# marbl/meryl

Hardware: AMD Instinct MI355X
Metric: distinct k-mers counted/sec (whole node) (higher is better)
Workload: dtype u64; 1 GPU; meryl count k=21 on synthetic short reads: 66666667 x 150 bp reads per GPU (10.00 Gbp per GPU, 30x of a 333333334 bp genome, 0.5% substitutions, 0.01% N), inputs resident in HBM; k=21, reads_per_gpu=66666667, bases_per_gpu=10066666717, n_distinct=1181289506, parallelism=1 GPU, transport=none (one GPU), n_instances=8648488363, w_prefix=18

## Files before the change

meryl_amd/csrc/mgc_api.cpp:

```cpp
#include "../../include/meryl_gpu_count.h"
#include "mgc_device.h"
#include "mgc_session.hpp"
#include "mgc_gzip_par.hpp"
#include "mgc_runs.hpp"
#include "mgc_selector.hpp"
#include "mgc_value.hpp"

#include <algorithm>
#include <cstdio>
#include <cstdlib>
#include <cstring>
#include <string>
#include <thread>
#include <vector>

namespace mgc {
std::string &thread_last_error() {
  thread_local std::string e;
  return e;
}

Switches read_switches() {
  Switches sw;
  auto off = [](const char *n) { const char *e = getenv(n); return e && e[0] == '0'; };
  auto on1 = [](const char *n) { const char *e = getenv(n); return e && e[0] == '1'; };
  auto num = [](const char *n, uint64_t d) { const char *e = getenv(n); return (e && *e) ? strtoull(e, nullptr, 10) : d; };
  sw.fine_hist = !off("MGC_FINE_HIST"); sw.hpc_msd = !off("MGC_HPC_MSD"); sw.hpc_digits = !off("MGC_HPC_DIGITS");
  sw.const_k = !off("MGC_KMER_CONST_K"); sw.packed_bases = !off("MGC_PACKED_BASES"); sw.narrow = !off("MGC_NARROW"); sw.wide_msd = !off("MGC_WIDE_MSD");
  sw.group_pipe = !off("MGC_GROUP_PIPE"); sw.soa5 = !off("MGC_SOA5"); sw.k96 = !off("MGC_K96"); sw.finish = !off("MGC_FINISH");
  sw.nolist = on1("MGC_FINISH_NOLIST");
  sw.finish_trace = getenv("MGC_FINISH_TRACE") != nullptr; sw.group_dbg = getenv("MGC_GROUP_DBG") != nullptr; sw.hash_dbg = getenv("MGC_HASH_DBG") != nullptr;
  { const char *e = getenv("MGC_HASH_MULTI"); sw.hash_multi = (e && *e) ? atoi(e) : -1; }
  { const char *e = getenv("MGC_HASH_STREAM"); sw.hash_stream = (e && *e) ? atoi(e) : -1; }
  sw.min_top = (uint32_t)num("MGC_FINISH_MIN_TOP", 0);
  sw.finish_target = num("MGC_FINISH_TARGET", 0);
  sw.stream_max = num("MGC_STREAM_MAX", (uint64_t)1 << 22);
  sw.bucket_bases = num("MGC_BUCKET_BASES", 0);
  sw.huge_streams = (uint32_t)num("MGC_HUGE_STREAMS", 4);
  sw.huge_slices = !off("MGC_HUGE_SLICES");
  sw.pass_stagger = (uint32_t)num("MGC_PASS_STAGGER", 0);
  sw.group_batch_bytes = num("MGC_GROUP_BATCH_BYTES", sw.group_batch_bytes);
  sw.group_batch_files = (uint32_t)num("MGC_GROUP_BATCH_FILES", 0);
  return sw;
}
}
using mgc::set_err;

namespace {


uint64_t number_of_bits64(uint64_t v) {
  uint64_t b = 0;
  while (v) { b++; v >>= 1; }
  return b;
}

uint64_t expected_simple_size(uint32_t k, uint64_t n_est, uint32_t suffix_len) {
  if (2 * k - 2 * suffix_len > 42) return UINT64_MAX;
  const uint64_t low_bits  = 16;
  const uint64_t n_entries = (uint64_t)1 << (2 * k - 2 * suffix_len);
  const uint64_t exp_max   = (uint64_t)(0.004 * (double)n_est);
  const uint64_t exp_bits  = number_of_bits64(exp_max) + 1;
  const uint64_t extra     = (exp_bits < low_bits) ? 0 : (exp_bits - low_bits);
  return (n_entries * low_bits + n_entries * extra) / 8;
}

void best_prefix_size(const mgc_count_config &c, uint64_t n_est, uint64_t mem_allowed, uint32_t *best,
                      uint64_t *mem_used) {
  const uint32_t k = c.k;
  const uint32_t seg_bits = c.page_size * 8, seg_bytes = c.page_size;
  *best = 0;
  *mem_used = UINT64_MAX;
  for (uint32_t wp = 1; wp < 2 * k - 1; wp++) {
    const uint64_t n_prefix = (uint64_t)1 << wp;
    const uint64_t kpp = n_est / n_prefix + 1;
    const uint64_t kps = seg_bits / (2 * k - wp);
    const uint64_t spp = kpp / kps + 1;
    if (wp + number_of_bits64(spp) + number_of_bits64(seg_bytes) >= 64) break;
    const uint64_t struct_mem = (uint64_t)c.sizeof_count_array * n_prefix + 8 * n_prefix * spp;
    const uint64_t data_min   = n_prefix * seg_bytes;
    const uint64_t total      = struct_mem + n_prefix * spp * seg_bytes;
    if (struct_mem + data_min > mem_allowed) break;
    if ((wp > 9) && (total + (uint64_t)16 * wp * 1024 * 1024 < *mem_used)) {
      *mem_used = total;
      *best = wp;
    }
    if (total > (uint64_t)16 * *mem_used) break;
  }
}

}

extern "C" uint32_t mgc_version(void) { return (0u << 16) | 3u; }

extern "C" int mgc_configure_counting(mgc_count_config *c) {
  if (!c) return MGC_EINVAL;
  if (c->k == 0 || c->k > 64) {
    set_err(nullptr, "ERROR: Kmer size not supplied with modifier k=<kmer-size>.");
    return MGC_EINVAL;
  }
  if (c->mode < 0 || c->mode > 2) return MGC_EINVAL;
  if (c->page_size == 0) c->page_size = 4096;
  if (c->sizeof_count_array == 0) c->sizeof_count_array = 3232;

  c->use_simple = 0; c->w_prefix = 0; c->n_prefix = 0; c->w_data = 0; c->n_batches = 1; c->memory_used = 0;

  const uint64_t mem_simple = expected_simple_size(c->k, c->n_kmers_estimate, c->count_suffix_length);
  uint64_t mem_complex = UINT64_MAX;
  uint32_t best = 0, n_batches = 1;

  if (c->k > 5) {
    for (n_batches = 1; mem_complex > c->memory_allowed; n_batches++) {
      best_prefix_size(*c, c->n_kmers_estimate / n_batches, c->memory_allowed, &best, &mem_complex);
      if (n_batches > (1u << 20)) {
        set_err(nullptr, "configureCounting: no prefix size fits in %lu bytes", (unsigned long)c->memory_allowed);
        return MGC_EINVAL;
      }
    }
    c->w_prefix = best;
    c->n_prefix = (uint64_t)1 << best;
    c->w_data   = 2 * c->k - best;
  }
  if ((mem_simple < mem_complex) && (mem_simple < c->memory_allowed)) {
    c->use_simple = 1; c->memory_used = mem_simple;
  } else {
// ... 1402 lines not shown
```

meryl_amd/csrc/mgc_count.cpp:

```cpp
#include "mgc_session.hpp"
#include "mgc_group_batch.hpp"
#include "mgc_group_route.hpp"

#include <algorithm>
#include <vector>

#define TRY(expr) do { const int rc__ = (expr); if (rc__ != MGC_OK) return rc__; } while (0)

namespace {
using S = mgc_session;

struct StageTimer {
  bool on;
  hipStream_t st;
  hipEvent_t ev[MGC_NUM_STAGES][2];
  bool used[MGC_NUM_STAGES];
  StageTimer(bool enable, hipStream_t s) : on(enable), st(s) {
    for (int i = 0; i < MGC_NUM_STAGES; i++) {
      used[i] = false;
      if (on) { (void)hipEventCreate(&ev[i][0]); (void)hipEventCreate(&ev[i][1]); }
    }
  }
  ~StageTimer() {
    if (on) for (int i = 0; i < MGC_NUM_STAGES; i++) { (void)hipEventDestroy(ev[i][0]); (void)hipEventDestroy(ev[i][1]); }
// ... 316 lines not shown
  std::vector<uint64_t> h_counts(nb);
  const bool wide_msd_on = sw.wide_msd && !c.homopoly_compress;
  if (!in.keys) {
    if (sw.packed_bases && n_bases) {
      const size_t pb = mgc::kp_packed_bytes(n_bases);
      bool room = s->buf[S::B_PACKED].cap >= pb;
      if (!room) {
        size_t free_b = 0, total_b = 0;
        room = hipMemGetInfo(&free_b, &total_b) == hipSuccess &&
               (double)free_b + (double)s->arena_bytes() >= (double)n_bases * (double)(2 + 14ull * kw) + (double)pb;
      }
      if (room) {
        if (s->ensure(S::B_PACKED, pb) == hipSuccess) d_packed = s->buf[S::B_PACKED].p;
        else (void)hipGetLastError();
      }
    }
    tm.begin(MGC_STAGE_HISTOGRAM);
    if (n_bases >= (1u << 22) && ((kw == 1 && 2 * k - bucket_bits <= 41) || wide_msd_on) && mgc::kmer_histogram_fine_ok(k, bucket_bits, s->sfx_mask, sw)) {
      HIP_TRY(s, s->ensure(S::B_FINE, sizeof(uint64_t) << 15));
      uint64_t *fine = reinterpret_cast<uint64_t *>(s->buf[S::B_FINE].p);
      HIP_TRY(s, mgc::launch_kmer_histogram_fine(d_bases, n_bases, k, c.mode, d_counts64, fine, part_ws, st, sw.const_k, 6, d_packed));
      d_fine = fine;
    } else if (c.homopoly_compress && n_bases >= (1u << 22) && (2 * k - bucket_bits) % 2 == 0 && 2 * k - bucket_bits >= 20 &&
               sw.hpc_digits && mgc::kmer_histogram_hpc_ok(k, bucket_bits, s->sfx_mask, sw)) {
      HIP_TRY(s, s->ensure(S::B_FINE, sizeof(uint64_t) * std::max<size_t>((size_t)1 << 15, mgc::kmer_histogram_hpc_entries(bucket_bits))));
      uint64_t *fine = reinterpret_cast<uint64_t *>(s->buf[S::B_FINE].p);
      HIP_TRY(s, mgc::launch_kmer_histogram_hpc(d_bases, n_bases, k, c.mode, bucket_bits, d_counts64, fine, part_ws, st, sw.const_k, d_packed));
      d_fine_hpc = fine;
    } else
    HIP_TRY(s, mgc::launch_kmer_histogram(d_bases, n_bases, k, c.mode, bucket_bits, d_counts64, part_ws, st, s->sfx_mask, s->sfx_test, d_packed));
    tm.end(MGC_STAGE_HISTOGRAM);
    prof.stage_launches[MGC_STAGE_HISTOGRAM] = 1;
    HIP_TRY(s, hipMemcpyAsync(h_counts.data(), d_counts64, sizeof(uint64_t) * nb, hipMemcpyDeviceToHost, st));
    HIP_TRY(s, hipStreamSynchronize(st));
  } else {
    memcpy(h_counts.data(), in.counts, sizeof(uint64_t) * nb);
    uint64_t n_ext = 0;
    for (uint32_t b = 0; b < nb; b++) n_ext += h_counts[b];
    if (in.fine && sw.fine_hist && bucket_bits <= 8 && n_ext >= (1u << 22) && s->sfx_mask == 0 && !c.homopoly_compress &&
        2 * k >= 15 + 2 && ((kw == 1 && 2 * k - bucket_bits <= 41) || wide_msd_on))
      d_fine = in.fine;
  }
  memset(s->file_instances, 0, sizeof(s->file_instances));
  for (uint32_t b = 0; b < nb; b++) {
    plan.files[b].size = h_counts[b];
    plan.files[b].start = h_meta[b] = N;
    N += h_counts[b];
    plan.max_bucket = std::max(plan.max_bucket, h_counts[b]);
    s->file_instances[b >> (bucket_bits - MGC_NUM_FILES_BITS)] += h_counts[b];
  }
  s->n_instances = N;
  plan.fine = d_fine != nullptr;
  plan.fine_hpc = d_fine_hpc != nullptr;
  return MGC_OK;
}

int Count::buffers() {
  mgc::make_sort_plan(0, rem_bits, &full);
  const bool odd = !use_finish && (full.num_passes & 1u) != 0;
  if (!in.keys) HIP_TRY(s, s->ensure(S::B_X, kbytes * N));
  y_base_bytes = kbytes * (odd ? N : plan.max_bucket);
  HIP_TRY(s, s->ensure(S::B_Y, y_base_bytes));
  X = in.keys ? reinterpret_cast<unsigned char *>(in.keys) : reinterpret_cast<unsigned char *>(s->buf[S::B_X].p);
  Y = reinterpret_cast<unsigned char *>(s->buf[S::B_Y].p);
  sort_ws_bytes = mgc::sort_workspace_bytes(plan.max_bucket) + 256;
  HIP_TRY(s, s->ensure(S::B_SORT_WS, sort_ws_bytes));
  sort_ws = s->buf[S::B_SORT_WS].p;
  d_err = reinterpret_cast<uint32_t *>(reinterpret_cast<unsigned char *>(sort_ws) + sort_ws_bytes - 256);
  HIP_TRY(s, hipMemsetAsync(d_err, 0, 32, st));
  if (s->profiling) {
    pass_ev.resize((size_t)nb * ev_per_file);
    for (auto &e : pass_ev) (void)hipEventCreate(&e);
  }
  return MGC_OK;
}

int Count::partition(bool soa, bool k96) {
  if (in.keys) return MGC_OK;
  HIP_TRY(s, hipMemcpyAsync(d_starts, h_meta.data(), sizeof(uint64_t) * nb, hipMemcpyHostToDevice, st));
  uint64_t *d_k96flags = d_starts + nb;
  if (k96) HIP_TRY(s, hipMemcpyAsync(d_k96flags, h_meta.data() + nb, sizeof(uint64_t) * nb, hipMemcpyHostToDevice, st));
  tm.begin(MGC_STAGE_PARTITION);
  HIP_TRY(s, mgc::launch_kmer_partition(d_bases, n_bases, k, c.mode, bucket_bits, d_starts, (void *)X, part_ws, st,
                                        s->sfx_mask, s->sfx_test, k96 ? d_k96flags : (soa ? d_counts64 : nullptr), sw.const_k, d_packed));
  tm.end(MGC_STAGE_PARTITION);
  const uint64_t packed_b = d_packed ? mgc::kp_packed_bytes(n_bases) : 0;
  prof.hist_bytes = n_bases + packed_b;
  prof.partition_bytes = d_packed ? packed_b : n_bases;
  for (uint32_t b = 0; b < nb; b++) prof.partition_bytes += plan.files[b].size * (soa ? 5u : ((k96 && plan.files[b].k96) ? 12u : (uint64_t)kbytes));
  prof.stage_launches[MGC_STAGE_PARTITION] = 2;
  return MGC_OK;
}

int Count::count_full() {
  TRY(partition(false, false));
  const bool odd = (full.num_passes & 1u) != 0;
  tm.begin(MGC_STAGE_SORT);
  for (uint32_t b = 0; b < nb; b++) {
    FilePlan &x = plan.files[b];
    if (x.size == 0) continue;
    void *alt = odd ? (void *)(Y + kbytes * x.start) : (void *)Y;
    int in_alt = 0;
    hipEvent_t *pe = s->profiling ? &pass_ev[(size_t)b * ev_per_file] : nullptr;
    HIP_TRY(s, mgc::launch_radix_sort(seg(b), alt, x.size, kw, full, sort_ws, sort_ws_bytes - 256, d_err, &in_alt, st, pe));
    x.passes = full.num_passes;
    sort_launch_groups++;
  }
  tm.end(MGC_STAGE_SORT);
  void *d_sorted = odd ? (void *)Y : (void *)X;

  HIP_TRY(s, s->ensure(S::B_RLE_WS, mgc::rle_workspace_bytes(N)));
  rle_ws = s->buf[S::B_RLE_WS].p;
  tm.begin(MGC_STAGE_RLE);
  HIP_TRY(s, mgc::launch_rle_count(d_sorted, N, kw, rle_ws, st));
  HIP_TRY(s, mgc::rle_read_total(rle_ws, &nd, st));
  s->n_distinct = nd;
  HIP_TRY(s, s->ensure(S::B_UNIQUE, kbytes * nd));
  HIP_TRY(s, s->ensure(S::B_COUNTS, sizeof(uint32_t) * nd));
  s->d_unique = s->buf[S::B_UNIQUE].p;
  s->d_counts = reinterpret_cast<uint32_t *>(s->buf[S::B_COUNTS].p);
  HIP_TRY(s, mgc::launch_rle_emit(d_sorted, N, kw, rle_ws, s->d_unique, s->d_counts, st));
  tm.end(MGC_STAGE_RLE);
  prof.stage_launches[MGC_STAGE_RLE] = 3;
  return MGC_OK;
}

int Count::finish_buffers() {
  const uint64_t ng_total = plan.ng_total;
  HIP_TRY(s, s->ensure(S::B_SUBSTART, sizeof(uint64_t) * (plan.ns_total + 1)));
  HIP_TRY(s, s->ensure(S::B_GROUPS, sizeof(uint64_t) * (ng_total + 2 + 3 * (uint64_t)nb)));
  HIP_TRY(s, s->ensure(S::B_LARGE, sizeof(uint32_t) * (ng_total + 1)));
  HIP_TRY(s, s->ensure(S::B_NONEMPTY, sizeof(uint32_t) * (ng_total + 1) + sizeof(uint64_t) * 2 * ((uint64_t)nb + 1)));
  HIP_TRY(s, s->ensure(S::B_GSCAN, mgc::finish_scan_scratch_bytes(ng_total + 1)));
  HIP_TRY(s, s->ensure(S::B_RLE_WS, mgc::rle_workspace_bytes(plan.max_bucket)));
  d_substart = reinterpret_cast<uint64_t *>(s->buf[S::B_SUBSTART].p);
  d_group    = reinterpret_cast<uint64_t *>(s->buf[S::B_GROUPS].p);
  d_stats    = d_group + ng_total + 1;
  d_large    = reinterpret_cast<uint32_t *>(s->buf[S::B_LARGE].p);
  d_retrycnt = reinterpret_cast<uint64_t *>(s->buf[S::B_NONEMPTY].p) + nb + 1;
  d_nz       = reinterpret_cast<uint32_t *>(d_retrycnt + nb + 1);
  HIP_TRY(s, hipMemsetAsync(s->buf[S::B_NONEMPTY].p, 0, sizeof(uint64_t) * 2 * ((size_t)nb + 1), st));
  HIP_TRY(s, hipMemsetAsync(d_group, 0, sizeof(uint64_t) * (ng_total + 1 + 3 * (size_t)nb), st));
  rle_ws = s->buf[S::B_RLE_WS].p;
  return MGC_OK;
}

int Count::prepare_headers() {
  if ((!d_fine && !d_fine_hpc) || nb > 256) return MGC_OK;
  uint64_t on[4] = {0, 0, 0, 0};
  size_t off = 0;
  bool any = false;
  for (uint32_t b = 0; b < nb; b++) {
    FilePlan &x = plan.files[b];
    x.nws_off = off;
    if (!msd_file(x)) continue;
    any = true;
    on[b >> 6] |= 1ull << (b & 63u);
    off += ((x.kind == Group::NARROW ? mgc::narrow_scratch_bytes(x.size) : mgc::wide_scratch_bytes(x.size, kw)) + 255) / 256 * 256;
  }
  if (!any) return MGC_OK;
  HIP_TRY(s, s->ensure(S::B_SORT_HDRS, hdr_bytes * nb));
  HIP_TRY(s, s->ensure(S::B_NARROW_WS, off));
  d_nhdrs = reinterpret_cast<unsigned char *>(s->buf[S::B_SORT_HDRS].p);
  d_nws = reinterpret_cast<unsigned char *>(s->buf[S::B_NARROW_WS].p);
  if (d_fine) TRY(narrow_prepare(probe, -1));
  else HIP_TRY(s, mgc::launch_hpc_prepare(d_fine_hpc, bucket_bits, on, d_nhdrs, st));
  HIP_TRY(s, hipMemsetAsync(d_nws, 0, off, st));
// ... 541 lines not shown
```

meryl_amd/csrc/mgc_device.h:

```cpp
#pragma once

#include <hip/hip_runtime.h>
#include <stddef.h>
#include <stdint.h>
#include "mgc_label.hpp"
#include "../../include/meryl_gpu_count.h"

namespace mgc {

struct Switches {
  bool fine_hist = true;
  bool hpc_msd = true;
  bool hpc_digits = true;
  bool const_k = true;
  bool packed_bases = true;
  bool narrow = true;
  bool wide_msd = true;
  bool soa5 = true;
  bool group_pipe = true;
  bool k96 = true;
  bool finish = true;
  bool nolist = false;
  bool finish_trace = false;
  bool group_dbg = false;
  uint32_t pass_stagger = 0;
  bool hash_dbg = false;
  int  hash_multi = -1;
  int  hash_stream = -1;
  uint32_t min_top = 0;
  uint64_t finish_target = 0;
  uint64_t stream_max = (uint64_t)1 << 22;
  bool     huge_slices = true;
  uint32_t huge_streams = 4;
  uint64_t bucket_bases = 0;
  uint64_t group_batch_bytes = (uint64_t)1 << 40;
  uint32_t group_batch_files = 0;
};
Switches read_switches();



constexpr int      KP_BLOCK       = 256;
constexpr int      KP_ITEMS       = 16;
constexpr int      KP_TILE        = KP_BLOCK * KP_ITEMS;
constexpr int      KP_MAX_BUCKETS = 1024;

uint32_t kp_grid_size(uint64_t n_bases, uint32_t bucket_bits);
size_t   kp_workspace_bytes(uint32_t bucket_bits);
size_t   kp_packed_bytes(uint64_t n_bases);

bool       kmer_histogram_fine_ok(uint32_t k, uint32_t bucket_bits, uint64_t sfx_mask, const Switches &sw);
bool       kmer_histogram_hpc_ok(uint32_t k, uint32_t bucket_bits, uint64_t sfx_mask, const Switches &sw);
uint32_t   kmer_histogram_hpc_entries(uint32_t bucket_bits);
hipError_t launch_kmer_histogram_hpc(const uint8_t *d_bases, uint64_t n_bases, uint32_t k, int mode, uint32_t bucket_bits,
                                     uint64_t *d_bucket_counts, uint64_t *d_fine_hist, void *d_ws, hipStream_t st, bool const_k = true ,
                                     void *d_packed = nullptr);
hipError_t launch_kmer_histogram_fine(const uint8_t *d_bases, uint64_t n_bases, uint32_t k, int mode, uint64_t *d_bucket_counts,
                                      uint64_t *d_fine_hist, void *d_ws, hipStream_t st, bool const_k = true ,
                                      uint32_t bucket_bits = 6 ,
                                      void *d_packed = nullptr);
bool       kmer_histogram_fine_bits_ok(uint32_t k, uint32_t bucket_bits);
hipError_t launch_kmer_histogram(const uint8_t *d_bases, uint64_t n_bases, uint32_t k, int mode,
                                 uint32_t bucket_bits, uint64_t *d_bucket_counts, void *d_ws, hipStream_t st,
                                 uint64_t sfx_mask = 0, uint64_t sfx_test = 0, void *d_packed = nullptr);
hipError_t launch_kmer_partition(const uint8_t *d_bases, uint64_t n_bases, uint32_t k, int mode,
                                 uint32_t bucket_bits, const uint64_t *d_bucket_starts, void *d_keys,
                                 void *d_ws, hipStream_t st, uint64_t sfx_mask = 0, uint64_t sfx_test = 0,
                                 const uint64_t *d_soa_counts = nullptr ,
                                 bool const_k = true , void *d_packed = nullptr);

struct SortPlan {
  uint32_t radix_bits;
  uint32_t block;
  uint32_t kpt;
  uint32_t tile;
  uint32_t mode;
  uint32_t hpc;
  uint32_t num_passes;
  uint32_t pass_shift[16];
  uint32_t pass_bits[16];
};

void   make_sort_plan(uint32_t begin_bit, uint32_t end_bit, SortPlan *plan);
void   make_hpc_group_plan(uint32_t low_bit, uint32_t passes, SortPlan *plan);
void   make_hpc_mixed_plan(uint32_t low_bit, SortPlan *plan);
size_t sort_workspace_bytes(uint64_t n);

hipError_t launch_radix_sort(void *d_keys, void *d_alt, uint64_t n, uint32_t key_words, const SortPlan &plan,
                             void *d_ws, size_t ws_bytes, uint32_t *d_error, int *result_in_alt,
                             hipStream_t st, hipEvent_t *pass_events );
size_t     sort_header_bytes();
enum class GroupKeys : uint32_t {
  U64,
  SOA5,
  K128,
  K96,
};
struct GroupFile {
  void *keys = nullptr, *alt = nullptr;
  uint64_t n = 0;
  const SortPlan *plan = nullptr;
  GroupKeys layout = GroupKeys::U64;
  uint32_t soa_hi_mask = 0;
  uint32_t *d_error = nullptr;
  uint64_t *d_sub_starts = nullptr;
  hipStream_t st = nullptr;
  hipEvent_t *pass_events = nullptr;
  void *prepared = nullptr, *scratch = nullptr;
  void *ws = nullptr; size_t ws_bytes = 0;
  bool pipe = false;
  uint32_t stagger = 0;
  bool dbg = false;
  uint32_t tr_a = 0, tr_b = 0;
};
bool       sort_plan_narrows(const SortPlan &plan, uint64_t n, uint32_t key_words, bool on = true );
size_t     narrow_scratch_bytes(uint64_t n);
hipError_t launch_narrow_prepare(const uint64_t *d_fine, uint32_t nb, const unsigned char *bits_a, const unsigned char *on, void *d_hdrs,
                                 hipStream_t st);
hipError_t launch_group_narrow(GroupFile &f);
struct GroupBatch {
  GroupFile *files = nullptr; uint32_t nfiles = 0;
  void *d_table = nullptr, *h_table = nullptr;
  uint32_t *d_ctl = nullptr;
  uint32_t *d_error = nullptr;
  hipStream_t st = nullptr;
  hipEvent_t *pass_events = nullptr;
};
size_t     group_batch_table_bytes(uint32_t nfiles);
hipError_t launch_group_narrow_batch(GroupBatch &b);
bool       sort_plan_wide_msd(const SortPlan &plan, uint64_t n, bool on = true );
hipError_t launch_hpc_prepare(const uint64_t *d_fine_hpc, uint32_t bucket_bits, const uint64_t on[4], void *d_hdrs, hipStream_t st);
size_t     wide_scratch_bytes(uint64_t n, uint32_t key_words);
hipError_t launch_group_wide(GroupFile &f);

size_t     rle_workspace_bytes(uint64_t n);
hipError_t launch_rle_count(const void *d_sorted, uint64_t n, uint32_t key_words, void *d_ws, hipStream_t st);
hipError_t rle_read_total(const void *d_ws, uint64_t *n_distinct, hipStream_t st);
hipError_t launch_rle_emit(const void *d_sorted, uint64_t n, uint32_t key_words, void *d_ws, void *d_unique,
                           uint32_t *d_counts, hipStream_t st, const uint64_t *d_out_base = nullptr);

uint64_t   finish_capacity_for(uint32_t key_words);
uint64_t   finish_target_for(uint32_t key_words, const Switches &sw);
bool       finish_stream_ok(uint32_t key_words, uint32_t low_bits, bool narrow = true);
uint64_t   finish_stream_capacity();
uint64_t   finish_stream_target(const Switches &sw);
uint64_t   finish_stream_distinct();
hipError_t launch_subbucket_bounds(const void *d_keys, uint64_t n, uint32_t key_words, uint32_t low, uint32_t top_bits,
                                   uint64_t *d_starts , uint64_t *d_max ,
                                   uint32_t *d_large_list ,
                                   uint64_t *d_large_count ,
                                   uint32_t *d_nonempty_list , uint64_t *d_nonempty_count ,
                                   hipStream_t st);
// ... 130 lines not shown
```

meryl_amd/csrc/mgc_kmer.hip:

```cpp
#include "mgc_common.hpp"
#include "mgc_bases.hpp"

namespace mgc {


__device__ __forceinline__ void encode16(uint4 v, u32 &codes, u32 &inval) { encode16(v.x, v.y, v.z, v.w, codes, inval); }

struct PackedBases { u32 *codes; unsigned short *inval; };

__device__ __forceinline__ u64 revcomp64(u64 f, u32 key_shift ) {
  u64 x = __brevll(f ^ 0xAAAAAAAAAAAAAAAAull);
  x = ((x >> 1) & 0x5555555555555555ull) | ((x & 0x5555555555555555ull) << 1);
  return x >> key_shift;
}

constexpr int KP_WORDS = KP_TILE / 16 + 4;

__device__ __forceinline__ void kp_stage_tile(const uint8_t *__restrict__ bases, u64 n, u64 tile0, bool aligned,
                                              u32 *s_codes, u32 *s_inval, PackedBases pk, bool last) {
  const u32 t = threadIdx.x;
  const u64 w0 = tile0 / 16;
  {
    u32 c, iv;
    encode16(load16(bases, tile0 + (u64)t * 16, n, aligned), c, iv);
// ... 314 lines not shown
        const u32 tpb = (u32)(KP_BLOCK * KH_NV) >> fbits, fr = tid / tpb, lr = tid % tpb, per_bucket = 1u << (KH_FINE_BITS - fbits);
        u32 rs = 0;
        for (u32 i = lr; i < per_bucket; i += tpb) rs += kh_fine[(fr << (KH_FINE_BITS - fbits)) + i];
        for (u32 o = tpb / 2; o > 0; o >>= 1) rs += __shfl_xor(rs, o);
        if (lr == 0) {
          const u32 c = rs - s_prev[fr];
          s_prev[fr] = rs;
          if (vwg < vgrid) block_hist[(vwg << fbits) + fr] = c;
          if (c) atomicAdd(&bucket_counts[fr], (u64)c);
        }
      }
    }
  }
  __syncthreads();
  for (u32 i = tid; i < TABLE; i += KP_BLOCK * KH_NV) {
    const u32 c = kh_fine[i];
    if (c) atomicAdd(&fine_hist[i], (u64)c);
  }
}

__global__ __launch_bounds__(256)
void kmer_scan_kernel(u64 *__restrict__ block_hist, u32 grid, u32 nb, const u64 *__restrict__ bucket_starts) {
  __shared__ u64 s_tmp[256 / 64 + 1];
  const u32 b = blockIdx.x;
  u64 carry = bucket_starts[b];
  for (u32 base = 0; base < grid; base += 256 * 8) {
    u64 v[8], sum = 0;
#pragma unroll
    for (int q = 0; q < 8; q++) {
      const u32 g = base + threadIdx.x * 8 + q;
      v[q] = (g < grid) ? block_hist[(u64)g * nb + b] : 0ull;
      sum += v[q];
    }
    u64 tot;
    u64 run = carry + block_excl_scan<256, u64>(sum, s_tmp, &tot);
#pragma unroll
    for (int q = 0; q < 8; q++) {
      const u32 g = base + threadIdx.x * 8 + q;
      if (g < grid) block_hist[(u64)g * nb + b] = run;
      run += v[q];
    }
    carry += tot;
  }
}

typedef __attribute__((address_space(1))) u32     kp_gu32;
typedef __attribute__((address_space(1))) uint8_t kp_gu8;
typedef __attribute__((address_space(1))) u64     kp_gu64;
typedef u32 kp_u32x3 __attribute__((ext_vector_type(3)));
typedef __attribute__((address_space(1))) __attribute__((aligned(4))) kp_u32x3 kp_gu32x3;
__device__ __forceinline__ void kp_gstore32(u64 addr, u32 v)     { *reinterpret_cast<kp_gu32 *>(addr) = v; }
__device__ __forceinline__ void kp_gstore8(u64 addr, uint8_t v)  { *reinterpret_cast<kp_gu8 *>(addr) = v; }
__device__ __forceinline__ void kp_gstore64(u64 addr, u64 v)     { *reinterpret_cast<kp_gu64 *>(addr) = v; }
__device__ __forceinline__ void kp_gstore96(u64 addr, u32 a, u32 b, u32 c) { kp_u32x3 v; v.x = a; v.y = b; v.z = c; *reinterpret_cast<kp_gu32x3 *>(addr) = v; }

template <typename K, int MAXB, bool SOA = false, int KC = 0, int BB = 6, bool PK = false>
__global__ __launch_bounds__(KP_BLOCK, (sizeof(K) == 16) ? 2 : 4)
void kmer_partition_kernel(const uint8_t *__restrict__ bases, u64 n, u32 k_arg, int mode_arg, u32 bucket_bits_arg,
                           u64 num_tiles, const u64 *__restrict__ block_base, K *__restrict__ out, u64 sfx_mask_arg, u64 sfx_test,
                           const u64 *__restrict__ soa_starts = nullptr, const u64 *__restrict__ soa_counts = nullptr,
                           u32 vgrid = 0 ,
                           PackedBases pk = PackedBases{nullptr, nullptr}) {
  const u32 k = KC ? (u32)KC : k_arg;
  const int mode = KC ? 0 : mode_arg;
  const u32 bucket_bits = KC ? (u32)BB : bucket_bits_arg;
  const u64 sfx_mask = KC ? 0ull : sfx_mask_arg;
  static_assert(KC == 0 || MAXB >= (1 << BB), "the buckets of a constant-k form fit its tables");
  extern __shared__ __attribute__((aligned(16))) unsigned char kp_dyn_smem[];
  K *s_keys = reinterpret_cast<K *>(kp_dyn_smem);
  __shared__ u64 s_cursor[MAXB];
  __shared__ u32 s_cnt[MAXB];
  __shared__ u32 s_base[MAXB];
  __shared__ u32 s_codes[KP_WORDS];
  __shared__ u32 s_inval[KP_WORDS];
  __shared__ u32 s_tmp[KP_BLOCK / 64 + 1];

  const u32  nb = 1u << bucket_bits;
  const u32  bucket_shift = 2 * k - bucket_bits;
  const bool aligned = ((reinterpret_cast<uintptr_t>(bases) & 15) == 0);
  const u32  tid = threadIdx.x;

  __shared__ u64 s_fstart[SOA ? MAXB : 1], s_fhi[SOA ? MAXB : 1];
  constexpr bool OB = MAXB <= 64;
  __shared__ u64 s_ob[OB ? MAXB : 1], s_ob_hi[SOA ? MAXB : 1];
  static_assert(!SOA || OB, "the 5-byte layout is a 64-file layout");
  if constexpr (SOA) {
    for (u32 b = tid; b < nb; b += KP_BLOCK) {
      s_fstart[b] = soa_starts[b];
      if constexpr (sizeof(K) == 8) s_fhi[b] = 8ull * soa_starts[b] + 4ull * soa_counts[b];
      else                          s_fhi[b] = soa_counts[b];
    }
  }

  const u32 nvirt = vgrid ? vgrid : gridDim.x;
  for (u32 vwg = blockIdx.x; vwg < nvirt; vwg += gridDim.x) {
  __syncthreads();
  for (u32 b = tid; b < nb; b += KP_BLOCK) s_cursor[b] = block_base[(u64)vwg * nb + b];
  u64 t_begin, t_end;
  kp_tile_range(num_tiles, t_begin, t_end, vwg, nvirt);

  uint4 nx = make_uint4(0, 0, 0, 0), nx_halo = make_uint4(0, 0, 0, 0);
  auto prefetch = [&](u64 tile) __attribute__((always_inline)) {
    if (tile >= t_end) return;
    if constexpr (PK) {
      const u64 w0 = tile * (u64)KP_BLOCK;
      nx.x = pk.codes[w0 + tid]; nx.y = pk.inval[w0 + tid];
      if (tid < 4) { nx_halo.x = pk.codes[w0 + KP_BLOCK + tid]; nx_halo.y = pk.inval[w0 + KP_BLOCK + tid]; }
    } else {
      nx = load16(bases, tile * KP_TILE + (u64)tid * 16, n, aligned);
      if (tid < 4) nx_halo = load16(bases, tile * KP_TILE + (u64)KP_TILE + (u64)tid * 16, n, aligned);
    }
  };
  prefetch(t_begin);
  for (u64 tile = t_begin; tile < t_end; tile++) {
    for (u32 b = tid; b < nb; b += KP_BLOCK) s_cnt[b] = 0;
    if constexpr (PK) {
      s_codes[tid] = nx.x; s_inval[tid] = nx.y;
      if (tid < 4) { s_codes[KP_BLOCK + tid] = nx_halo.x; s_inval[KP_BLOCK + tid] = nx_halo.y; }
    } else {
      u32 c, iv;
      encode16(nx, c, iv);
      s_codes[tid] = c; s_inval[tid] = iv;
      if (tid < 4) { encode16(nx_halo, c, iv); s_codes[KP_BLOCK + tid] = c; s_inval[KP_BLOCK + tid] = iv; }
    }
    prefetch(tile + 1);
    __syncthreads();

    K keys[KP_ITEMS];
    const u32 vmask = kp_suffix_filter(keys, kp_thread_kmers(s_codes, s_inval, k, mode, keys), sfx_mask, sfx_test);
    u32 total = 0;

    if (nb == 1) {
      const u32 c = __popc(vmask);
      const u32 base = block_excl_scan<KP_BLOCK, u32>(c, s_tmp, &total);
      u32 o = base;
#pragma unroll
      for (int j = 0; j < KP_ITEMS; j++)
        if ((vmask >> j) & 1u) s_keys[o++] = keys[j];
      if (tid == 0) { s_base[0] = 0; s_cnt[0] = total; if constexpr (OB) s_ob[0] = reinterpret_cast<u64>(out) + (u64)sizeof(K) * s_cursor[0]; }
      __syncthreads();
    } else {
      u32 ranks[KP_ITEMS];
#pragma unroll
      for (int j = 0; j < KP_ITEMS; j++) {
        ranks[j] = 0;
        if ((vmask >> j) & 1u) ranks[j] = atomicAdd(&s_cnt[KeyOps<K>::bucket(keys[j], bucket_shift)], 1u);
      }
      __syncthreads();
      u32 v[4], sum = 0;
#pragma unroll
      for (int q = 0; q < 4; q++) {
        const u32 b = tid * 4 + q;
        v[q] = (b < nb) ? s_cnt[b] : 0u;
        sum += v[q];
      }
      u32 run = block_excl_scan<KP_BLOCK, u32>(sum, s_tmp, &total);
#pragma unroll
      for (int q = 0; q < 4; q++) {
        const u32 b = tid * 4 + q;
        if (b < nb) {
          s_base[b] = run;
          if constexpr (SOA && sizeof(K) == 8) {
            const u64 rel0 = s_cursor[b] - s_fstart[b] - (u64)run;
            s_ob[b]    = reinterpret_cast<u64>(out) + 8ull * s_fstart[b] + 4ull * rel0;
            s_ob_hi[b] = reinterpret_cast<u64>(out) + s_fhi[b] + rel0;
          } else if constexpr (SOA) {
            const u64 rel0 = s_cursor[b] - s_fstart[b] - (u64)run;
            s_ob[b] = (reinterpret_cast<u64>(out) + 16ull * s_fstart[b] + (s_fhi[b] ? 12ull : 16ull) * rel0) | (s_fhi[b] ? 1ull : 0ull);
          } else if constexpr (OB) {
            s_ob[b] = reinterpret_cast<u64>(out) + (u64)sizeof(K) * (s_cursor[b] - (u64)run);
          }
        }
        run += v[q];
      }
      __syncthreads();
#pragma unroll
      for (int j = 0; j < KP_ITEMS; j++)
        if ((vmask >> j) & 1u) s_keys[s_base[KeyOps<K>::bucket(keys[j], bucket_shift)] + ranks[j]] = keys[j];
      __syncthreads();
    }

    for (u32 i = tid; i < total; i += KP_BLOCK) {
      const K   key = s_keys[i];
      const u32 b   = (nb == 1) ? 0u : KeyOps<K>::bucket(key, bucket_shift);
      if constexpr (SOA && sizeof(K) == 8) {
        kp_gstore32(s_ob[b] + 4ull * i, (u32)KeyOps<K>::low64(key));
        kp_gstore8(s_ob_hi[b] + (u64)i, (uint8_t)(KeyOps<K>::low64(key) >> 32));
      }
      else if constexpr (SOA) {
        const u64 ob = s_ob[b];
        const bool f96 = (ob & 1ull) != 0;
        const u64 addr = (ob & ~1ull) + (u64)(f96 ? 12u : 16u) * i;
        kp_gstore96(addr, (u32)key.lo, (u32)(key.lo >> 32), (u32)key.hi);
        if (!f96) kp_gstore32(addr + 12ull, (u32)(key.hi >> 32));
      }
      else if constexpr (OB) {
        if constexpr (sizeof(K) == 8) kp_gstore64(s_ob[b] + 8ull * i, (u64)KeyOps<K>::low64(key));
        else *reinterpret_cast<K *>(s_ob[b] + (u64)sizeof(K) * i) = key;
      }
      else out[s_cursor[b] + (u64)(i - s_base[b])] = key;
    }
    __syncthreads();
    for (u32 b = tid; b < nb; b += KP_BLOCK) s_cursor[b] += s_cnt[b];
    __syncthreads();
  }
  }
}

static int kmer_const_k(uint32_t k, int mode, bool on) {
  if (!on || mode != 0) return 0;
  return (k == 21 || k == 31 || k == 51) ? (int)k : 0;
}

constexpr uint32_t KP_VGRID = 16384, KP_PHYS = 2048;
static uint32_t kp_vgrid_max(uint32_t bucket_bits) {
  static const uint32_t env = [] { const char *e = getenv("MGC_PART_VGRID"); return (e && *e) ? (uint32_t)atoi(e) : 0u; }();
  if (bucket_bits > 8) return KP_PHYS;
  return (env >= 256 && env <= KP_VGRID) ? env : KP_PHYS;
}
uint32_t kp_grid_size(uint64_t n_bases, uint32_t bucket_bits) {
  const uint64_t num_tiles = (n_bases + KP_TILE - 1) / KP_TILE;
  const uint64_t vmax = kp_vgrid_max(bucket_bits);
  uint64_t g = num_tiles < vmax ? num_tiles : vmax;
  return (uint32_t)(g ? g : 1);
}

size_t kp_workspace_bytes(uint32_t bucket_bits) {
  return (size_t)(bucket_bits > 8 ? KP_PHYS : KP_VGRID) * ((size_t)1 << bucket_bits) * sizeof(uint64_t);
}

static uint64_t kp_packed_words(uint64_t n_bases) { return (n_bases + KP_TILE - 1) / KP_TILE * (uint64_t)KP_BLOCK + 4; }
size_t kp_packed_bytes(uint64_t n_bases) { return (size_t)(kp_packed_words(n_bases) * 6); }
static PackedBases kp_packed(void *d_packed, uint64_t n_bases) {
  if (!d_packed) return PackedBases{nullptr, nullptr};
  u32 *codes = reinterpret_cast<u32 *>(d_packed);
  return PackedBases{codes, reinterpret_cast<unsigned short *>(codes + kp_packed_words(n_bases))};
}

hipError_t launch_kmer_histogram(const uint8_t *d_bases, uint64_t n_bases, uint32_t k, int mode,
                                 uint32_t bucket_bits, uint64_t *d_bucket_counts, void *d_ws, hipStream_t st,
                                 uint64_t sfx_mask, uint64_t sfx_test, void *d_packed) {
  const PackedBases pk = kp_packed(d_packed, n_bases);
  const uint32_t nb = 1u << bucket_bits;
  MGC_CHECK(hipMemsetAsync(d_bucket_counts, 0, sizeof(uint64_t) * nb, st));
  if (n_bases == 0) return hipSuccess;
  const uint64_t num_tiles = (n_bases + KP_TILE - 1) / KP_TILE;
  const uint32_t grid = kp_grid_size(n_bases, bucket_bits);
  if (k <= 32)
    hipLaunchKernelGGL(kmer_hist_kernel<u64>, dim3(grid), dim3(KP_BLOCK), 0, st,
                       d_bases, (u64)n_bases, k, mode, bucket_bits, (u64)num_tiles,
                       reinterpret_cast<u64 *>(d_ws), reinterpret_cast<u64 *>(d_bucket_counts), (u64)sfx_mask, (u64)sfx_test, pk);
  else
    hipLaunchKernelGGL(kmer_hist_kernel<K128>, dim3(grid), dim3(KP_BLOCK), 0, st,
                       d_bases, (u64)n_bases, k, mode, bucket_bits, (u64)num_tiles,
                       reinterpret_cast<u64 *>(d_ws), reinterpret_cast<u64 *>(d_bucket_counts), (u64)sfx_mask, (u64)sfx_test, pk);
  return hipGetLastError();
}

bool kmer_histogram_fine_ok(uint32_t k, uint32_t bucket_bits, uint64_t sfx_mask, const Switches &sw) {
  return sw.fine_hist && k <= 64 && 2 * k >= (uint32_t)KH_FINE_BITS + 2 && bucket_bits == 6 && sfx_mask == 0;
}
bool kmer_histogram_fine_bits_ok(uint32_t k, uint32_t bucket_bits) { return k <= 64 && 2 * k >= (uint32_t)KH_FINE_BITS + 2 && bucket_bits >= 6 && bucket_bits <= 8; }

struct KhLaunch {
  const uint8_t *d_bases; uint64_t n_bases; uint32_t k; int mode; uint64_t num_tiles; uint32_t vgrid;
  void *d_ws; uint64_t *d_bucket_counts, *d_fine_hist; uint32_t fbits, nvp; hipStream_t st; PackedBases pk;
};
template <int HB, int KC>
static hipError_t kh_launch_form(const KhLaunch &a) {
  constexpr size_t LDS = sizeof(u32) * (HB ? hpc_table_size(HB) : (1u << KH_FINE_BITS));
  static const hipError_t raised = hipFuncSetAttribute(reinterpret_cast<const void *>(&kmer_hist_fine_kernel<HB, KC>),
                                                       hipFuncAttributeMaxDynamicSharedMemorySize, (int)LDS);
  (void)raised;
  hipLaunchKernelGGL((kmer_hist_fine_kernel<HB, KC>), dim3((a.vgrid + a.nvp - 1) / a.nvp), dim3(KP_BLOCK * KH_NV), LDS, a.st,
                     a.d_bases, (u64)a.n_bases, a.k, a.mode, (u64)a.num_tiles, a.vgrid, reinterpret_cast<u64 *>(a.d_ws),
                     reinterpret_cast<u64 *>(a.d_bucket_counts), reinterpret_cast<u64 *>(a.d_fine_hist), a.fbits, a.nvp, a.pk);
  return hipGetLastError();
}
static hipError_t kh_prepare(const uint8_t *d_bases, uint64_t n_bases, uint32_t k, int mode, uint32_t bucket_bits, uint64_t *d_bucket_counts,
                             uint64_t *d_fine_hist, size_t fine_entries, void *d_ws, hipStream_t st, void *d_packed, KhLaunch *a) {
  MGC_CHECK(hipMemsetAsync(d_bucket_counts, 0, sizeof(uint64_t) << bucket_bits, st));
  MGC_CHECK(hipMemsetAsync(d_fine_hist, 0, sizeof(uint64_t) * fine_entries, st));
  const uint32_t vgrid = kp_grid_size(n_bases, bucket_bits);
  const uint32_t nvp = std::max<uint32_t>((uint32_t)KH_NV, (vgrid + 511u) / 512u);
  *a = KhLaunch{d_bases, n_bases, k, mode, (n_bases + KP_TILE - 1) / KP_TILE, vgrid, d_ws, d_bucket_counts, d_fine_hist, 6u, nvp, st,
                kp_packed(d_packed, n_bases)};
  return hipSuccess;
}

hipError_t launch_kmer_histogram_fine(const uint8_t *d_bases, uint64_t n_bases, uint32_t k, int mode, uint64_t *d_bucket_counts,
                                      uint64_t *d_fine_hist, void *d_ws, hipStream_t st, bool const_k, uint32_t bucket_bits,
                                      void *d_packed) {
  if (bucket_bits < 6 || bucket_bits > 8) return hipErrorInvalidValue;
  KhLaunch a;
  MGC_CHECK(kh_prepare(d_bases, n_bases, k, mode, bucket_bits, d_bucket_counts, d_fine_hist, (size_t)1 << KH_FINE_BITS, d_ws, st, d_packed, &a));
  if (n_bases == 0) return hipSuccess;
  a.fbits = bucket_bits;
  switch (kmer_const_k(k, mode, const_k)) {
    case 21: return kh_launch_form<0, 21>(a);
    case 31: return kh_launch_form<0, 31>(a);
    case 51: return kh_launch_form<0, 51>(a);
    default: return kh_launch_form<0, 0>(a);
  }
}

bool kmer_histogram_hpc_ok(uint32_t k, uint32_t bucket_bits, uint64_t sfx_mask, const Switches &sw) {
  return sw.hpc_msd && (bucket_bits == 6 || bucket_bits == 8) && k <= 64 && 2 * k >= bucket_bits + 10 + 2 && sfx_mask == 0;
}
uint32_t kmer_histogram_hpc_entries(uint32_t bucket_bits) { return hpc_table_size((int)(bucket_bits / 2 + 5)); }

hipError_t launch_kmer_histogram_hpc(const uint8_t *d_bases, uint64_t n_bases, uint32_t k, int mode, uint32_t bucket_bits,
                                     uint64_t *d_bucket_counts, uint64_t *d_fine_hist, void *d_ws, hipStream_t st, bool const_k,
                                     void *d_packed) {
  if (bucket_bits != 6 && bucket_bits != 8) return hipErrorInvalidValue;
  KhLaunch a;
  MGC_CHECK(kh_prepare(d_bases, n_bases, k, mode, bucket_bits, d_bucket_counts, d_fine_hist, kmer_histogram_hpc_entries(bucket_bits), d_ws, st, d_packed, &a));
  if (n_bases == 0) return hipSuccess;
  const bool k31 = kmer_const_k(k, mode, const_k) == 31;
  if (bucket_bits == 6) return k31 ? kh_launch_form<8, 31>(a) : kh_launch_form<8, 0>(a);
  return k31 ? kh_launch_form<9, 31>(a) : kh_launch_form<9, 0>(a);
}

struct KpLaunch {
  const uint8_t *d_bases; uint64_t n_bases; uint32_t k; int mode; uint32_t bucket_bits; uint64_t num_tiles;
  void *d_ws, *d_keys; uint64_t sfx_mask, sfx_test; const u64 *soa_starts, *soa_counts; uint32_t rows, grid; hipStream_t st;
  PackedBases pk;
};
template <typename K, int MAXB, bool SOA, int KC, int BB, bool PK>
static void kp_launch_form(const KpLaunch &a) {
  if constexpr (sizeof(K) == 16) {
    static bool attr_done = false;
    if (!attr_done) {
      (void)hipFuncSetAttribute(reinterpret_cast<const void *>(&kmer_partition_kernel<K, MAXB, SOA, KC, BB, PK>),
                                hipFuncAttributeMaxDynamicSharedMemorySize, (int)(KP_TILE * sizeof(K)));
      attr_done = true;
    }
  }
  hipLaunchKernelGGL((kmer_partition_kernel<K, MAXB, SOA, KC, BB, PK>), dim3(a.grid), dim3(KP_BLOCK), KP_TILE * sizeof(K), a.st,
                     a.d_bases, (u64)a.n_bases, a.k, a.mode, a.bucket_bits, (u64)a.num_tiles, reinterpret_cast<const u64 *>(a.d_ws),
                     reinterpret_cast<K *>(a.d_keys), (u64)a.sfx_mask, (u64)a.sfx_test, a.soa_starts, a.soa_counts, a.rows, a.pk);
}
template <typename K, int MAXB, bool SOA, int KC, int BB = 6>
static void kp_launch(const KpLaunch &a) {
  if (a.pk.codes) kp_launch_form<K, MAXB, SOA, KC, BB, true>(a);
  else            kp_launch_form<K, MAXB, SOA, KC, BB, false>(a);
}

hipError_t launch_kmer_partition(const uint8_t *d_bases, uint64_t n_bases, uint32_t k, int mode,
                                 uint32_t bucket_bits, const uint64_t *d_bucket_starts, void *d_keys,
                                 void *d_ws, hipStream_t st, uint64_t sfx_mask, uint64_t sfx_test, const uint64_t *d_soa_counts, bool const_k,
                                 void *d_packed) {
  if (n_bases == 0) return hipSuccess;
  const uint32_t nb = 1u << bucket_bits;
  const uint64_t num_tiles = (n_bases + KP_TILE - 1) / KP_TILE;
  const uint32_t rows = kp_grid_size(n_bases, bucket_bits);
  const uint32_t grid = rows < KP_PHYS ? rows : KP_PHYS;
  hipLaunchKernelGGL(kmer_scan_kernel, dim3(nb), dim3(256), 0, st,
                     reinterpret_cast<u64 *>(d_ws), rows, nb, reinterpret_cast<const u64 *>(d_bucket_starts));
  MGC_CHECK(hipGetLastError());
  const KpLaunch a{d_bases, n_bases, k, mode, bucket_bits, num_tiles, d_ws, d_keys, sfx_mask, sfx_test, nullptr, nullptr, rows, grid, st,
                   kp_packed(d_packed, n_bases)};
  const int kck = (sfx_mask == 0) ? kmer_const_k(k, mode, const_k) : 0;
  if (d_soa_counts) {
    if (!(nb == 64 && sfx_mask == 0 && k <= 51)) return hipErrorInvalidValue;
    KpLaunch s = a;
    s.soa_starts = reinterpret_cast<const u64 *>(d_bucket_starts); s.soa_counts = reinterpret_cast<const u64 *>(d_soa_counts);
    if (k > 32) { if (kck == 51) kp_launch<K128, 64, true, 51>(s); else kp_launch<K128, 64, true, 0>(s); }
    else        { if (kck == 21) kp_launch<u64, 64, true, 21>(s);  else kp_launch<u64, 64, true, 0>(s); }
    return hipGetLastError();
  }
  if (nb == 256 && kck == 31) kp_launch<u64, 256, false, 31, 8>(a);
  else if (nb == 64 && kck == 21) kp_launch<u64, 64, false, 21>(a);
  else if (nb == 64 && kck == 31) kp_launch<u64, 64, false, 31>(a);
  else if (nb == 64 && kck == 51) kp_launch<K128, 64, false, 51>(a);
  else if (k <= 32) { if (nb <= 64) kp_launch<u64, 64, false, 0>(a);  else kp_launch<u64, KP_MAX_BUCKETS, false, 0>(a); }
  else              { if (nb <= 64) kp_launch<K128, 64, false, 0>(a); else kp_launch<K128, KP_MAX_BUCKETS, false, 0>(a); }
  return hipGetLastError();
}



hipError_t warm_kmer() { hipFuncAttributes a; return hipFuncGetAttributes(&a, reinterpret_cast<const void *>(&kmer_scan_kernel)); }

}
```

Measured before the change: 12.52 billion distinct k-mers/s.

## Add dedicated 5-byte partition kernel with optional two-block tiles

Moves the 5-byte (SOA, k<=32) partition path out of the generic templated kernel into a dedicated kernel. The new kernel stores keys in shared memory as 32-bit low parts plus 16-bit high parts instead of full 64-bit keys, and computes the bucket prefix with a single-wavefront shuffle scan. It defaults to tiles of two 4096-base blocks with 512 threads, which halves the number of per-tile synchronisations and scans at the cost of lower occupancy per block. It also adds an environment knob to pick one- or two-block tiles, and it now rejects k outside 20..23 on this path.

```diff
diff --git a/meryl_amd/csrc/mgc_api.cpp b/meryl_amd/csrc/mgc_api.cpp
--- a/meryl_amd/csrc/mgc_api.cpp
+++ b/meryl_amd/csrc/mgc_api.cpp
@@ -41,6 +41,7 @@
   sw.pass_stagger = (uint32_t)num("MGC_PASS_STAGGER", 0);
   sw.group_batch_bytes = num("MGC_GROUP_BATCH_BYTES", sw.group_batch_bytes);
   sw.group_batch_files = (uint32_t)num("MGC_GROUP_BATCH_FILES", 0);
+  { const uint64_t t = num("MGC_PART_TILE", 0); if (t == (uint64_t)mgc::KP_TILE || t == 2ull * mgc::KP_TILE) sw.part_tile = (uint32_t)t; }
   return sw;
 }
 }
diff --git a/meryl_amd/csrc/mgc_count.cpp b/meryl_amd/csrc/mgc_count.cpp
--- a/meryl_amd/csrc/mgc_count.cpp
+++ b/meryl_amd/csrc/mgc_count.cpp
@@ -422,7 +422,8 @@
   if (k96) HIP_TRY(s, hipMemcpyAsync(d_k96flags, h_meta.data() + nb, sizeof(uint64_t) * nb, hipMemcpyHostToDevice, st));
   tm.begin(MGC_STAGE_PARTITION);
   HIP_TRY(s, mgc::launch_kmer_partition(d_bases, n_bases, k, c.mode, bucket_bits, d_starts, (void *)X, part_ws, st,
-                                        s->sfx_mask, s->sfx_test, k96 ? d_k96flags : (soa ? d_counts64 : nullptr), sw.const_k, d_packed));
+                                        s->sfx_mask, s->sfx_test, k96 ? d_k96flags : (soa ? d_counts64 : nullptr), sw.const_k, d_packed,
+                                        sw.part_tile));
   tm.end(MGC_STAGE_PARTITION);
   const uint64_t packed_b = d_packed ? mgc::kp_packed_bytes(n_bases) : 0;
   prof.hist_bytes = n_bases + packed_b;
diff --git a/meryl_amd/csrc/mgc_device.h b/meryl_amd/csrc/mgc_device.h
--- a/meryl_amd/csrc/mgc_device.h
+++ b/meryl_amd/csrc/mgc_device.h
@@ -8,6 +8,7 @@
 
 namespace mgc {
 
+constexpr uint32_t KP_PART_TILE = 8192;
 struct Switches {
   bool fine_hist = true;
   bool hpc_msd = true;
@@ -17,6 +18,7 @@
   bool narrow = true;
   bool wide_msd = true;
   bool soa5 = true;
+  uint32_t part_tile = KP_PART_TILE;
   bool group_pipe = true;
   bool k96 = true;
   bool finish = true;
@@ -44,6 +46,7 @@
 constexpr int      KP_ITEMS       = 16;
 constexpr int      KP_TILE        = KP_BLOCK * KP_ITEMS;
 constexpr int      KP_MAX_BUCKETS = 1024;
+static_assert(KP_PART_TILE == 2 * KP_TILE, "the 5-byte layout's partition: two blocks per tile, 512 threads");
 
 uint32_t kp_grid_size(uint64_t n_bases, uint32_t bucket_bits);
 size_t   kp_workspace_bytes(uint32_t bucket_bits);
@@ -67,7 +70,8 @@
                                  uint32_t bucket_bits, const uint64_t *d_bucket_starts, void *d_keys,
                                  void *d_ws, hipStream_t st, uint64_t sfx_mask = 0, uint64_t sfx_test = 0,
                                  const uint64_t *d_soa_counts = nullptr ,
-                                 bool const_k = true , void *d_packed = nullptr);
+                                 bool const_k = true , void *d_packed = nullptr,
+                                 uint32_t part_tile = KP_PART_TILE );
 
 struct SortPlan {
   uint32_t radix_bits;
diff --git a/meryl_amd/csrc/mgc_kmer.hip b/meryl_amd/csrc/mgc_kmer.hip
--- a/meryl_amd/csrc/mgc_kmer.hip
+++ b/meryl_amd/csrc/mgc_kmer.hip
@@ -420,13 +420,12 @@
 
   __shared__ u64 s_fstart[SOA ? MAXB : 1], s_fhi[SOA ? MAXB : 1];
   constexpr bool OB = MAXB <= 64;
-  __shared__ u64 s_ob[OB ? MAXB : 1], s_ob_hi[SOA ? MAXB : 1];
-  static_assert(!SOA || OB, "the 5-byte layout is a 64-file layout");
+  __shared__ u64 s_ob[OB ? MAXB : 1];
+  static_assert(!SOA || (OB && sizeof(K) == 16), "SOA here: the K96 records of a 64-file layout (the 5-byte layout: kmer_partition5_kernel)");
   if constexpr (SOA) {
     for (u32 b = tid; b < nb; b += KP_BLOCK) {
       s_fstart[b] = soa_starts[b];
-      if constexpr (sizeof(K) == 8) s_fhi[b] = 8ull * soa_starts[b] + 4ull * soa_counts[b];
-      else                          s_fhi[b] = soa_counts[b];
+      s_fhi[b] = soa_counts[b];
     }
   }
 
@@ -498,11 +497,7 @@
         const u32 b = tid * 4 + q;
         if (b < nb) {
           s_base[b] = run;
-          if constexpr (SOA && sizeof(K) == 8) {
-            const u64 rel0 = s_cursor[b] - s_fstart[b] - (u64)run;
-            s_ob[b]    = reinterpret_cast<u64>(out) + 8ull * s_fstart[b] + 4ull * rel0;
-            s_ob_hi[b] = reinterpret_cast<u64>(out) + s_fhi[b] + rel0;
-          } else if constexpr (SOA) {
+          if constexpr (SOA) {
             const u64 rel0 = s_cursor[b] - s_fstart[b] - (u64)run;
             s_ob[b] = (reinterpret_cast<u64>(out) + 16ull * s_fstart[b] + (s_fhi[b] ? 12ull : 16ull) * rel0) | (s_fhi[b] ? 1ull : 0ull);
           } else if constexpr (OB) {
@@ -521,11 +516,7 @@
     for (u32 i = tid; i < total; i += KP_BLOCK) {
       const K   key = s_keys[i];
       const u32 b   = (nb == 1) ? 0u : KeyOps<K>::bucket(key, bucket_shift);
-      if constexpr (SOA && sizeof(K) == 8) {
-        kp_gstore32(s_ob[b] + 4ull * i, (u32)KeyOps<K>::low64(key));
-        kp_gstore8(s_ob_hi[b] + (u64)i, (uint8_t)(KeyOps<K>::low64(key) >> 32));
-      }
-      else if constexpr (SOA) {
+      if constexpr (SOA) {
         const u64 ob = s_ob[b];
         const bool f96 = (ob & 1ull) != 0;
         const u64 addr = (ob & ~1ull) + (u64)(f96 ? 12u : 16u) * i;
@@ -542,6 +533,120 @@
     for (u32 b = tid; b < nb; b += KP_BLOCK) s_cursor[b] += s_cnt[b];
     __syncthreads();
   }
+  }
+}
+
+struct __attribute__((aligned(16))) KpOb5 { u64 lo, hi; };
+template <int KC, bool PK, int TB>
+__global__ __launch_bounds__(KP_BLOCK * TB, 4 / TB)
+void kmer_partition5_kernel(const uint8_t *__restrict__ bases, u64 n, u32 k_arg, int mode_arg, u64 num_blocks,
+                            const u64 *__restrict__ block_base, unsigned char *__restrict__ out,
+                            const u64 *__restrict__ soa_starts, const u64 *__restrict__ soa_counts, u32 vgrid, PackedBases pk) {
+  static_assert(TB == 1 || TB == 2, "tiles of one or two 4096-base blocks");
+  constexpr u32 NT = KP_BLOCK * TB, TILE = KP_TILE * TB, NF = 64;
+  const u32 k = KC ? (u32)KC : k_arg;
+  const int mode = KC ? 0 : mode_arg;
+  const u32 hi_shift = 2 * k - 38;
+  extern __shared__ __attribute__((aligned(16))) unsigned char kp_dyn_smem[];
+  u32 *s_lo = reinterpret_cast<u32 *>(kp_dyn_smem);
+  unsigned short *s_hi = reinterpret_cast<unsigned short *>(s_lo + TILE);
+  __shared__ u64 s_cursor[NF], s_f4[NF], s_f1[NF];
+  __shared__ KpOb5 s_ob[NF];
+  __shared__ u32 s_cnt[NF], s_base[NF], s_total;
+  __shared__ u32 s_codes[NT + 4], s_inval[NT + 4];
+  const bool aligned = ((reinterpret_cast<uintptr_t>(bases) & 15) == 0);
+  const u32  tid = threadIdx.x;
+  if (tid < NF) {
+    s_f4[tid] = 4ull * soa_starts[tid];
+    s_f1[tid] = 7ull * soa_starts[tid] + 4ull * soa_counts[tid];
+  }
+
+  const u32 nvirt = vgrid ? vgrid : gridDim.x;
+  for (u32 vwg = blockIdx.x; vwg < nvirt; vwg += gridDim.x) {
+    __syncthreads();
+    if (tid < NF) { s_cursor[tid] = block_base[(u64)vwg * NF + tid]; s_cnt[tid] = 0; }
+    u64 b_begin, b_end;
+    kp_tile_range(num_blocks, b_begin, b_end, vwg, nvirt);
+
+    uint4 nx = make_uint4(0, 0, 0, 0), nx_halo = make_uint4(0, 0, 0, 0);
+    auto prefetch = [&](u64 blk) __attribute__((always_inline)) {
+      if (blk >= b_end) return;
+      const u32 live = (TB == 1 || b_end - blk >= (u64)TB) ? NT : (u32)KP_BLOCK;
+      if constexpr (PK) {
+        const u64 w0 = blk * (u64)KP_BLOCK;
+        if (tid < live) { nx.x = pk.codes[w0 + tid]; nx.y = pk.inval[w0 + tid]; }
+        if (tid < 4) { nx_halo.x = pk.codes[w0 + live + tid]; nx_halo.y = pk.inval[w0 + live + tid]; }
+      } else {
+        if (tid < live) nx = load16(bases, blk * KP_TILE + (u64)tid * 16, n, aligned);
+        if (tid < 4) nx_halo = load16(bases, blk * KP_TILE + (u64)live * 16 + (u64)tid * 16, n, aligned);
+      }
+    };
+    prefetch(b_begin);
+    for (u64 blk = b_begin; blk < b_end; blk += TB) {
+      const u32 live = (TB == 1 || b_end - blk >= (u64)TB) ? NT : (u32)KP_BLOCK;
+      if constexpr (PK) {
+        if (tid < live) { s_codes[tid] = nx.x; s_inval[tid] = nx.y; }
+        if (tid < 4) { s_codes[live + tid] = nx_halo.x; s_inval[live + tid] = nx_halo.y; }
+      } else {
+        u32 c, iv;
+        if (tid < live) { encode16(nx, c, iv); s_codes[tid] = c; s_inval[tid] = iv; }
+        if (tid < 4) { encode16(nx_halo, c, iv); s_codes[live + tid] = c; s_inval[live + tid] = iv; }
+      }
+      prefetch(blk + TB);
+      __syncthreads();
+
+      u32 lo[KP_ITEMS], hi[KP_ITEMS], ranks[KP_ITEMS];
+      u32 vmask;
+      {
+        u64 keys[KP_ITEMS];
+        vmask = kp_thread_kmers(s_codes, s_inval, k, mode, keys);
+        if (TB > 1 && tid >= live) vmask = 0;
+#pragma unroll
+        for (int j = 0; j < KP_ITEMS; j++) { lo[j] = (u32)keys[j]; hi[j] = (u32)(keys[j] >> 32); }
+      }
+#pragma unroll
+      for (int j = 0; j < KP_ITEMS; j++) {
+        ranks[j] = 0;
+        if ((vmask >> j) & 1u) ranks[j] = atomicAdd(&s_cnt[hi[j] >> hi_shift], 1u);
+      }
+      __syncthreads();
+      if (tid < NF) {
+        const u32 cnt = s_cnt[tid];
+        u32 incl = cnt;
+#pragma unroll
+        for (int d = 1; d < 64; d <<= 1) {
+          const u32 y = __shfl_up(incl, d);
+          if ((int)tid >= d) incl += y;
+        }
+        const u32 run = incl - cnt;
+        const u64 cur = s_cursor[tid];
+        const u64 c0 = cur - (u64)run;
+        KpOb5 ob;
+        ob.lo = reinterpret_cast<u64>(out) + s_f4[tid] + 4ull * c0;
+        ob.hi = reinterpret_cast<u64>(out) + s_f1[tid] + c0;
+        s_ob[tid] = ob;
+        s_base[tid] = run;
+        s_cursor[tid] = cur + cnt;
+        s_cnt[tid] = 0;
+        if (tid == NF - 1) s_total = incl;
+      }
+      __syncthreads();
+      const u32 total = s_total;
+#pragma unroll
+      for (int j = 0; j < KP_ITEMS; j++)
+        if ((vmask >> j) & 1u) {
+          const u32 p = s_base[hi[j] >> hi_shift] + ranks[j];
+          s_lo[p] = lo[j]; s_hi[p] = (unsigned short)hi[j];
+        }
+      __syncthreads();
+
+      for (u32 i = tid; i < total; i += NT) {
+        const u32 l = s_lo[i], h = s_hi[i];
+        const KpOb5 ob = s_ob[h >> hi_shift];
+        kp_gstore32(ob.lo + 4ull * i, l);
+        kp_gstore8(ob.hi + (u64)i, (uint8_t)h);
+      }
+    }
   }
 }
 
@@ -684,10 +789,24 @@
   else            kp_launch_form<K, MAXB, SOA, KC, BB, false>(a);
 }
 
+template <int KC, bool PK, int TB>
+static void kp_launch5_form(const KpLaunch &a) {
+  const uint32_t grid = std::max<uint32_t>(1u, std::min<uint32_t>(a.rows, KP_PHYS / TB));
+  hipLaunchKernelGGL((kmer_partition5_kernel<KC, PK, TB>), dim3(grid), dim3(KP_BLOCK * TB), (size_t)KP_TILE * TB * 6, a.st,
+                     a.d_bases, (u64)a.n_bases, a.k, a.mode, (u64)a.num_tiles, reinterpret_cast<const u64 *>(a.d_ws),
+                     reinterpret_cast<unsigned char *>(a.d_keys), a.soa_starts, a.soa_counts, a.rows, a.pk);
+}
+template <int KC>
+static void kp_launch5(const KpLaunch &a, uint32_t tile) {
+  const bool two = tile == 2u * KP_TILE;
+  if (a.pk.codes) { if (two) kp_launch5_form<KC, true, 2>(a);  else kp_launch5_form<KC, true, 1>(a); }
+  else            { if (two) kp_launch5_form<KC, false, 2>(a); else kp_launch5_form<KC, false, 1>(a); }
+}
+
 hipError_t launch_kmer_partition(const uint8_t *d_bases, uint64_t n_bases, uint32_t k, int mode,
                                  uint32_t bucket_bits, const uint64_t *d_bucket_starts, void *d_keys,
                                  void *d_ws, hipStream_t st, uint64_t sfx_mask, uint64_t sfx_test, const uint64_t *d_soa_counts, bool const_k,
-                                 void *d_packed) {
+                                 void *d_packed, uint32_t part_tile) {
   if (n_bases == 0) return hipSuccess;
   const uint32_t nb = 1u << bucket_bits;
   const uint64_t num_tiles = (n_bases + KP_TILE - 1) / KP_TILE;
@@ -704,7 +823,10 @@
     KpLaunch s = a;
     s.soa_starts = reinterpret_cast<const u64 *>(d_bucket_starts); s.soa_counts = reinterpret_cast<const u64 *>(d_soa_counts);
     if (k > 32) { if (kck == 51) kp_launch<K128, 64, true, 51>(s); else kp_launch<K128, 64, true, 0>(s); }
-    else        { if (kck == 21) kp_launch<u64, 64, true, 21>(s);  else kp_launch<u64, 64, true, 0>(s); }
+    else {
+      if (k < 20 || k > 23 || (part_tile != (uint32_t)KP_TILE && part_tile != 2u * KP_TILE)) return hipErrorInvalidValue;
+      if (kck == 21) kp_launch5<21>(s, part_tile); else kp_launch5<0>(s, part_tile);
+    }
     return hipGetLastError();
   }
   if (nb == 256 && kck == 31) kp_launch<u64, 256, false, 31, 8>(a);
```

Result: no change. 12.61 billion distinct k-mers/s, median of 6 (+0.7%).
